# shahruk10/kaldi-tflite

Hardware: AMD Instinct MI355X
Metric: x-vectors/sec (10 s @16 kHz) (higher is better)
Workload: dtype f16mx

## Files before the change

include/ktf_hip.h:

```cpp
#ifndef KTF_HIP_H_
#define KTF_HIP_H_

#include <stddef.h>
#include <stdint.h>

#ifdef __cplusplus
extern "C" {
#endif

#define KTF_OK 0
#define KTF_EINVAL (-1)
#define KTF_ELAUNCH (-2)
#define KTF_EUNSUPPORTED (-3)

#define KTF_F32 0
#define KTF_BF16 1
#define KTF_BF16P 3

#define KTF_GEMM_F32 0
#define KTF_GEMM_BF16 1
#define KTF_GEMM_BF16X3 2
#define KTF_GEMM_F16MX 5
#define KTF_GEMM_BF16X4 6

// ... 104 lines not shown
    int64_t lds_bytes;
    int32_t nsplit;
    int32_t lds_form;
} KtfVcPlan;
int ktf_vad_cmvn_plan(int64_t B, int64_t T, int32_t D, int64_t ldo, KtfVcPlan* plan);
int ktf_cmvn_plan(int64_t T, int32_t D, int64_t ldo, KtfVcPlan* plan);

int ktf_route_short(const int32_t* lens, int64_t B, int32_t min_frames, int32_t* lens_main, int32_t* lens_short, int32_t* host_flag,
                    int32_t seq, void* stream);

typedef struct KtfTdnnDesc {
    int32_t units;
    int32_t din;
    int32_t din_pad;
    int32_t nctx;
    int32_t ctx[16];
    int32_t subsampling;
    int32_t valid;
    int32_t act;
    int32_t gemm;
    int32_t x_dtype, w_dtype, y_dtype;
    int32_t flags;
} KtfTdnnDesc;

#define KTF_TDNN_REF_TILES 1
#define KTF_TDNN_DET_STATS 2
#define KTF_TDNN_K_INTERLEAVED 4
#define KTF_TDNN_W_TILED 8

#define KTF_TDNN_MX_LOADER (1 << 24)

const char* ktf_tdnn_last_kernel(void);


int64_t ktf_tdnn_out_len(int64_t len, const KtfTdnnDesc* d);
int ktf_tdnn_out_lens(const int32_t* lens, int64_t B, const KtfTdnnDesc* d, int32_t* out_lens, void* stream);

int ktf_tdnn(const void* x, int64_t B, int64_t T, int64_t ldx, const int32_t* lens, const KtfTdnnDesc* d,
             const void* w, const void* w_lo, const float* bias, const float* scale, const float* shift,
             void* y, int64_t ldy, int32_t* out_lens, void* stream);

int ktf_tdnn_stats(const void* x, int64_t B, int64_t T, int64_t ldx, const int32_t* lens, const KtfTdnnDesc* d,
                   const void* w, const void* w_lo, const float* bias, const float* scale, const float* shift, double* sums,
                   void* stream);
int ktf_tdnn_split(const void* x_hi, const void* x_lo, int64_t B, int64_t T, int64_t ldx, const int32_t* lens,
                   const KtfTdnnDesc* d, const void* w, const void* w_lo, const float* bias, const float* scale,
                   const float* shift, void* y, void* y_lo, int64_t ldy, int32_t* out_lens, void* stream);
int ktf_tdnn_split_flat(const void* x_hi, const void* x_lo, int64_t B, int64_t T, int64_t ldx, const int32_t* row_starts, const int32_t* row_map,
                        const KtfTdnnDesc* d, const void* w, const void* w_lo, const float* bias, const float* scale,
                        const float* shift, void* y, void* y_lo, int64_t ldy, void* stream);
int64_t ktf_flat_stats_slots(int64_t T);
int64_t ktf_flat_row_map_rows(int64_t B, int64_t T);
int ktf_flat_row_map(const int32_t* row_starts, int64_t B, int64_t T, int32_t* map, void* stream);
int ktf_tdnn_split_flat_stats(const void* x_hi, const void* x_lo, int64_t B, int64_t T, int64_t ldx, const int32_t* row_starts,
                              const int32_t* row_map, const KtfTdnnDesc* d, const void* w, const void* w_lo, const float* bias, const float* scale,
                              const float* shift, double* sums, void* stream);
int ktf_stats_finalize_flat(const double* sums, int64_t slots, const int32_t* row_starts, int64_t T, int64_t B, int32_t D,
                            int32_t include_std, float eps, float* out, int64_t ld_out, void* stream);
int ktf_tdnn_split_stats(const void* x_hi, const void* x_lo, int64_t B, int64_t T, int64_t ldx, const int32_t* lens,
                         const KtfTdnnDesc* d, const void* w, const void* w_lo, const float* bias, const float* scale,
                         const float* shift, double* sums, void* stream);
int ktf_split_bf16(const float* src, int64_t rows, int32_t D, int64_t ld_src, void* hi, void* lo, int64_t ld_dst,
                   void* stream);
int ktf_split_bf16_rows(const float* src, int64_t B, int64_t T, int32_t D, int64_t ld_src, const int32_t* lens, void* hi, void* lo,
                        int64_t ld_dst, void* stream);
int ktf_mx_planes(const float* src, int64_t B, int64_t T, int32_t D, int64_t ld_src, const int32_t* lens, void* xh, void* xl4,
                  void* x4, void* xs, void* stream);
int ktf_tdnn_mx(const void* xh, const void* xl4, const void* x4, const void* xs, int64_t B, int64_t T, const int32_t* lens,
                const KtfTdnnDesc* d, const void* wh, const void* wq, const float* bias, const float* scale, const float* shift,
                void* yh, void* yl4, void* y4, void* ys, float* yf, int64_t ldy, void* stream);
int ktf_tdnn_mx_flat(const void* xh, const void* xl4, const void* x4, const void* xs, int64_t B, int64_t T, const int32_t* row_starts,
                     const int32_t* row_map, const KtfTdnnDesc* d, const void* wh, const void* wq, const float* bias, const float* scale,
                     const float* shift, void* yh, void* yl4, void* y4, void* ys, void* stream);
int ktf_tdnn_mx_flat_stats(const void* xh, const void* xl4, const void* x4, const void* xs, int64_t B, int64_t T, const int32_t* row_starts,
                           const int32_t* row_map, const KtfTdnnDesc* d, const void* wh, const void* wq, const float* bias, const float* scale,
                           const float* shift, double* sums, void* stream);
int ktf_tdnn_mx_stats(const void* xh, const void* xl4, const void* x4, const void* xs, int64_t B, int64_t T, const int32_t* lens,
                      const KtfTdnnDesc* d, const void* wh, const void* wq, const float* bias, const float* scale,
                      const float* shift, double* sums, void* stream);
int ktf_stats_finalize(const double* sums, const int32_t* lens, int64_t T, int64_t B, int32_t D, int32_t include_std,
                       float eps, float* out, int64_t ld_out, void* stream);
int64_t ktf_stats_slots(int64_t T);
int64_t ktf_tdnn_stats_slots(int64_t T, int32_t gemm);
int32_t ktf_tdnn_slot_rows(int32_t gemm);
int64_t ktf_mx_stats_slots(int64_t T, int32_t flags);
int32_t ktf_mx_slot_rows(int32_t flags);
int ktf_stats_finalize_slots(const double* sums, int64_t slots, int32_t slot_rows, const int32_t* lens, int64_t T, int64_t B, int32_t D,
                             int32_t include_std, float eps, float* out, int64_t ld_out, void* stream);

int ktf_activation_f32(float* y, int64_t B, int64_t T, int32_t D, int64_t ld, const int32_t* lens, int32_t act, const float* scale,
                       const float* shift, void* stream);

int ktf_affine_act_f32(const float* x, int64_t rows, int32_t D, int32_t act, const float* scale, const float* shift,
                       float* y, void* stream);
int ktf_convert_pad(const void* src, int32_t src_dtype, int64_t rows, int32_t D, int64_t ld_src, void* dst,
                    int32_t dst_dtype, int64_t ld_dst, void* stream);

int ktf_stats_pool(const void* x, int32_t x_dtype, int64_t B, int64_t T, int32_t D, int64_t ldx,
                   const int32_t* lens, int32_t input_period, int32_t include_std, float eps, float* out,
                   int64_t ld_out, void* stream);
int ktf_stats_pool_windowed_f32(const float* x, int64_t B, int64_t T, int32_t D, int32_t left, int32_t right,
                                int32_t input_period, int32_t output_period, int32_t start, int64_t T_out,
                                int32_t include_std, float eps, float* out, void* stream);

int ktf_xvec_tail_f32(const float* pooled, int64_t ld_pooled, const double* sums, int64_t slots, int32_t slot_rows, const int32_t* lens, int64_t T,
                      int64_t B, int32_t D, int32_t include_std, float eps, const float* W, int64_t ldw, const float* bias,
// ... 187 lines not shown
```

kaldi-tflite_amd/csrc/tdnn_mx.hip:

```cpp
#include "tdnn_mx_common.h"

#define MXP_ROWS 256
__global__ __launch_bounds__(MXP_ROWS) void mx_planes_kernel(const float* __restrict__ src, int64_t T, int64_t ld, int D,
                                                             const int32_t* __restrict__ lens, char* __restrict__ xh,
                                                             char* __restrict__ xl4, char* __restrict__ x4, char* __restrict__ xs) {
    __shared__ float tile[MXP_ROWS * 33];
    const int b = blockIdx.z, c = blockIdx.y, nch = gridDim.y;
    const int64_t t0 = (int64_t)blockIdx.x * MXP_ROWS;
    const int64_t len = lens ? (int64_t)lens[b] : T;
    if (t0 >= len) return;
    const int rows = (int)(len - t0 < MXP_ROWS ? len - t0 : MXP_ROWS);
    const int tid = threadIdx.x;
    const float* base = src + ((int64_t)b * T + t0) * ld + c * 32;
    const bool vec = (ld & 3) == 0 && ((uintptr_t)src & 15) == 0 && c * 32 + 32 <= ld;
#pragma unroll
    for (int k = 0; k < 8; ++k) {
        const int q = k * MXP_ROWS + tid, r = q >> 3, e4 = (q & 7) * 4;
        if (r < rows) {
            float v[4];
            if (vec) {
                const f32x4 t = *reinterpret_cast<const f32x4*>(base + (int64_t)r * ld + e4);
                const int nd = D - (c * 32 + e4);
                v[0] = nd > 0 ? t.x : 0.0f; v[1] = nd > 1 ? t.y : 0.0f; v[2] = nd > 2 ? t.z : 0.0f; v[3] = nd > 3 ? t.w : 0.0f;
            } else {
#pragma unroll
                for (int e = 0; e < 4; ++e) v[e] = (c * 32 + e4 + e < D) ? base[(int64_t)r * ld + e4 + e] : 0.0f;
            }
#pragma unroll
            for (int e = 0; e < 4; ++e) tile[r * 33 + e4 + e] = __builtin_amdgcn_fmed3f(v[e], -65504.0f, 65504.0f);
        }
    }
    __syncthreads();
    const int64_t rec0 = ((int64_t)b * nch + c) * T + t0;
    u32x4 hp[4];
    if (tid < rows) {
        float v[32];
#pragma unroll
        for (int e = 0; e < 32; ++e) v[e] = tile[tid * 33 + e];
        u32x4 l4, h4;
        unsigned sw;
        mx_encode32(v, hp, l4, h4, sw);
        *reinterpret_cast<u32x4*>(xl4 + (rec0 + tid) * 16) = l4;
        *reinterpret_cast<u32x4*>(x4 + (rec0 + tid) * 16) = h4;
        *reinterpret_cast<unsigned*>(xs + (rec0 + tid) * 4) = sw;
    }
    __syncthreads();
    unsigned* himg = reinterpret_cast<unsigned*>(tile);
    if (tid < rows) {
#pragma unroll
        for (int k = 0; k < 4; ++k) *reinterpret_cast<u32x4*>(himg + tid * 20 + k * 4) = hp[k];
    }
    __syncthreads();
#pragma unroll
    for (int k = 0; k < 4; ++k) {
        const int q = k * MXP_ROWS + tid, r = q >> 2;
        if (r < rows)
            *reinterpret_cast<u32x4*>(xh + rec0 * 64 + (int64_t)q * 16) = *reinterpret_cast<const u32x4*>(himg + r * 20 + (q & 3) * 4);
    }
}

extern "C" int ktf_mx_planes(const float* src, int64_t B, int64_t T, int32_t D, int64_t ld_src, const int32_t* lens, void* xh,
                             void* xl4, void* x4, void* xs, void* stream) {
    KTF_REQUIRE(B >= 0 && T >= 0 && D > 0 && ld_src >= D, "ktf_mx_planes: bad size");
    if (B == 0 || T == 0) return KTF_OK;
    KTF_REQUIRE(src && xh && xl4 && x4 && xs, "ktf_mx_planes: null argument");
    const int nch = (D + 31) / 32;
    KTF_REQUIRE(B < 65536 && nch < 65536, "ktf_mx_planes: B and D / 32 must be below 65536");
    hipLaunchKernelGGL(mx_planes_kernel, dim3((unsigned)((T + MXP_ROWS - 1) / MXP_ROWS), (unsigned)nch, (unsigned)B), dim3(MXP_ROWS), 0,
                       (hipStream_t)stream, src, T, ld_src, (int)D, lens, (char*)xh, (char*)xl4, (char*)x4, (char*)xs);
    KTF_CHECK_LAUNCH("ktf_mx_planes");
    return KTF_OK;
}

template <int ACT, int OUT, bool PADK, bool FLAT = false>
__device__ __forceinline__ void mx_tile(const MxParams& p, const int id, int mtiles, int ntiles, int gtiles, double* __restrict__ stats,
                                        unsigned char* rsm) {
    static_assert(!FLAT || OUT != MX_OUT_F32, "flat row tiles: plane output or fused pooling");
#define MX_ARG_BATCH()                                                                                                                     \
    asm volatile("" ::"s"(p.xh), "s"(p.wh), "s"(p.T), "s"(p.nss), "s"(p.nk), "s"(p.nctx), "s"(p.nch_in), "s"(p.ctx_pk[0]), "s"(p.ctx_pk[1]), \
                 "s"(p.t_div_m), "s"(p.t_div_s), "s"(p.start), "s"(p.sub), "s"(p.cut))
    const int xcd = id & 7, slot = id >> 3;
    const int g = (slot / ntiles) * 8 + xcd;
    const int nt = slot - (slot / ntiles) * ntiles;
    if (g >= gtiles) return;
    const int b = FLAT ? 0 : g / mtiles, mt = FLAT ? g : g - b * mtiles;
    const int n0 = nt * 256, t0 = FLAT ? 0 : mt * 256;
    const int tid = threadIdx.x, lane = tid & 63;
    const int wave = __builtin_amdgcn_readfirstlane(tid >> 6);
    const int wm = wave >> 2, wn = wave & 3;
    const int R0 = mt * 256;
    int len, out_len;
    [[maybe_unused]] bool dense = false;
    if constexpr (FLAT) {
        const int total = p.row_starts[mtiles];
        MX_ARG_BATCH();
        if (R0 >= total) return;
        len = (int)p.T;
        out_len = total - R0 < 256 ? total - R0 : 256;
        dense = total == mtiles * len;
    } else {
        len = p.lens ? p.lens[b] : (int)p.T;
        MX_ARG_BATCH();
        out_len = len - p.cut - p.start <= 0 ? 0 : (len - p.cut - p.start + p.sub - 1) / p.sub;
        if (t0 >= out_len) return;
    }
    const int lenm1 = len - 1;
    const int64_t ub = FLAT ? 0 : (int64_t)b * p.nch_in * p.T;
    const int nkp = p.nss * 4;
    const __amdgpu_buffer_rsrc_t r_xh = mx_rsrc_pinned(p.xh + (ub - MX_KQ_BIAS) * 64);
    const __amdgpu_buffer_rsrc_t r_wh = mx_rsrc_pinned(p.wh + (int64_t)nt * nkp * MX_TILE);
    const __amdgpu_buffer_rsrc_t r_wq = mx_rsrc_pinned(p.wq + (int64_t)nt * p.nss * MX_WQ_BLOCK);

    unsigned a_cb[2];
    int a_row[2];
#pragma unroll
    for (int i = 0; i < 2; ++i) {
        const int q = i * 512 + tid;
        const int row = q >> 2;
        a_cb[i] = (unsigned)(((q & 3) ^ ((4 - ((row >> 2) & 3)) & 3)) * 16);
        a_row[i] = p.start + (t0 + row) * p.sub;
    }
    [[maybe_unused]] int a_lm1[2] = {lenm1, lenm1}, s_lm1 = lenm1;
    int s_row = p.start + (t0 + lane + 64 * (wave & 3)) * p.sub;
// ... 428 lines not shown
```

kaldi-tflite_amd/kaldi_tflite_amd/_lib.py:

```python

import ctypes as C
import threading
import os

_HERE = os.path.dirname(os.path.abspath(__file__))
_OVERRIDE = os.environ.get("KTF_LIBRARY") if os.environ.get("KTF_ALLOW_LIBRARY_OVERRIDE") == "1" else None
LIB_PATH = _OVERRIDE or os.path.join(_HERE, "libktf_hip.so")

KTF_F32, KTF_BF16, KTF_BF16P = 0, 1, 3
PAIR = "bf16p"
GEMM_F32, GEMM_BF16, GEMM_BF16X3, GEMM_F16MX, GEMM_BF16X4 = 0, 1, 2, 5, 6
ACT_NONE, ACT_RELU, ACT_SIGMOID, ACT_TANH = 0, 1, 2, 3
(ACT_ELU, ACT_SELU, ACT_SOFTPLUS, ACT_SOFTSIGN, ACT_SWISH, ACT_GELU, ACT_EXPONENTIAL, ACT_HARD_SIGMOID,
 ACT_SOFTMAX) = range(4, 13)
TDNN_REF_TILES, TDNN_DET_STATS, TDNN_K_INTERLEAVED, TDNN_W_TILED = 1, 2, 4, 8
TAIL_SKIP_EMPTY = 1
TDNN_MX_LOADER = 1 << 24

IN_WAV, IN_FRAMES, IN_WINDOWED, IN_WAV_I16 = 0, 1, 2, 3
OUT_FRAMES, OUT_WINDOWED, OUT_FBANK, OUT_MFCC = 0, 1, 2, 3


class KtfBackendError(RuntimeError):
    pass
# ... 28 lines not shown


class VadCfg(C.Structure):
    _fields_ = [("energy_threshold", C.c_float), ("energy_mean_scale", C.c_float), ("proportion_threshold", C.c_float),
                ("frames_context", C.c_int32), ("energy_coeff", C.c_int32)]


class CmvnCfg(C.Structure):
    _fields_ = [("window", C.c_int32), ("norm_vars", C.c_int32), ("valid", C.c_int32), ("reserved", C.c_int32)]


class VcPlan(C.Structure):
    _fields_ = [("pos_ints", C.c_int64), ("stage_floats", C.c_int64), ("bs_floats", C.c_int64), ("col_floats", C.c_int64),
                ("lds_bytes", C.c_int64), ("nsplit", C.c_int32), ("lds_form", C.c_int32)]


class TdnnDesc(C.Structure):
    _fields_ = [("units", C.c_int32), ("din", C.c_int32), ("din_pad", C.c_int32), ("nctx", C.c_int32),
                ("ctx", C.c_int32 * 16), ("subsampling", C.c_int32), ("valid", C.c_int32), ("act", C.c_int32),
                ("gemm", C.c_int32), ("x_dtype", C.c_int32), ("w_dtype", C.c_int32), ("y_dtype", C.c_int32),
                ("flags", C.c_int32)]


_P = C.c_void_p
_i64, _i32, _f32, _u64 = C.c_int64, C.c_int32, C.c_float, C.c_uint64

PROTOTYPES = {
    "ktf_version": (_i32, []),
    "ktf_last_error": (C.c_size_t, [C.c_char_p, C.c_size_t]),
    "ktf_build_id": (C.c_char_p, []),
    "ktf_clock_probe": (C.c_int, [_P, _i64, _P]),
    "ktf_num_frames": (_i64, [_i64, _i32, _i32]),
    "ktf_num_frames_padded": (_i64, [_i64, _i32, _i32, _i32]),
    "ktf_frontend_f32": (C.c_int, [_P, _i64, _i64, _i32, C.POINTER(FrontendCfg), C.POINTER(FrontendTables), _i32, _P, _P, _u64, _P]),
    "ktf_dct_f32": (C.c_int, [_P, _i64, _i32, _i32, _P, _P, _P, _P]),
    "ktf_vad_mask_f32": (C.c_int, [_P, _i64, _i64, _i32, C.POINTER(VadCfg), _P, _P]),
    "ktf_vad_index": (C.c_int, [_P, _i64, _i64, _i32, C.POINTER(VadCfg), _P, _P, _P]),
    "ktf_cmvn_f32": (C.c_int, [_P, _i64, _i64, _i32, _i64, _P, C.POINTER(CmvnCfg), _P, _i64, _P, _P, _P]),
    "ktf_vad_cmvn": (C.c_int, [_P, _i64, _i64, _i32, C.POINTER(VadCfg), C.POINTER(CmvnCfg), _P, _i32, _i64, _P, _P, _P, _P]),
    "ktf_vad_cmvn_plan": (C.c_int, [_i64, _i64, _i32, _i64, C.POINTER(VcPlan)]),
    "ktf_cmvn_plan": (C.c_int, [_i64, _i32, _i64, C.POINTER(VcPlan)]),
    "ktf_route_short": (C.c_int, [_P, _i64, _i32, _P, _P, _P, _i32, _P]),
    "ktf_tdnn_out_len": (_i64, [_i64, C.POINTER(TdnnDesc)]),
    "ktf_tdnn_out_lens": (C.c_int, [_P, _i64, C.POINTER(TdnnDesc), _P, _P]),
    "ktf_tdnn_last_kernel": (C.c_char_p, []),
    "ktf_tdnn": (C.c_int, [_P, _i64, _i64, _i64, _P, C.POINTER(TdnnDesc), _P, _P, _P, _P, _P, _P, _i64, _P, _P]),
    "ktf_tdnn_stats": (C.c_int, [_P, _i64, _i64, _i64, _P, C.POINTER(TdnnDesc), _P, _P, _P, _P, _P, _P, _P]),
    "ktf_tdnn_split": (C.c_int, [_P, _P, _i64, _i64, _i64, _P, C.POINTER(TdnnDesc), _P, _P, _P, _P, _P, _P, _P, _i64, _P, _P]),
    "ktf_tdnn_split_flat": (C.c_int, [_P, _P, _i64, _i64, _i64, _P, _P, C.POINTER(TdnnDesc), _P, _P, _P, _P, _P, _P, _P, _i64, _P]),
    "ktf_tdnn_split_stats": (C.c_int, [_P, _P, _i64, _i64, _i64, _P, C.POINTER(TdnnDesc), _P, _P, _P, _P, _P, _P, _P]),
    "ktf_tdnn_split_flat_stats": (C.c_int, [_P, _P, _i64, _i64, _i64, _P, _P, C.POINTER(TdnnDesc), _P, _P, _P, _P, _P, _P, _P]),
    "ktf_flat_row_map_rows": (_i64, [_i64, _i64]),
    "ktf_flat_row_map": (C.c_int, [_P, _i64, _i64, _P, _P]),
    "ktf_flat_stats_slots": (_i64, [_i64]),
    "ktf_stats_finalize_flat": (C.c_int, [_P, _i64, _P, _i64, _i64, _i32, _i32, _f32, _P, _i64, _P]),
    "ktf_split_bf16": (C.c_int, [_P, _i64, _i32, _i64, _P, _P, _i64, _P]),
    "ktf_split_bf16_rows": (C.c_int, [_P, _i64, _i64, _i32, _i64, _P, _P, _P, _i64, _P]),
    "ktf_mx_planes": (C.c_int, [_P, _i64, _i64, _i32, _i64, _P, _P, _P, _P, _P, _P]),
    "ktf_tdnn_mx": (C.c_int, [_P, _P, _P, _P, _i64, _i64, _P, C.POINTER(TdnnDesc), _P, _P, _P, _P, _P, _P, _P, _P, _P, _P, _i64, _P]),
    "ktf_tdnn_mx_flat": (C.c_int, [_P, _P, _P, _P, _i64, _i64, _P, _P, C.POINTER(TdnnDesc), _P, _P, _P, _P, _P, _P, _P, _P, _P, _P]),
    "ktf_tdnn_mx_flat_stats": (C.c_int, [_P, _P, _P, _P, _i64, _i64, _P, _P, C.POINTER(TdnnDesc), _P, _P, _P, _P, _P, _P, _P]),
    "ktf_tdnn_mx_stats": (C.c_int, [_P, _P, _P, _P, _i64, _i64, _P, C.POINTER(TdnnDesc), _P, _P, _P, _P, _P, _P, _P]),
    "ktf_stats_finalize": (C.c_int, [_P, _P, _i64, _i64, _i32, _i32, _f32, _P, _i64, _P]),
    "ktf_stats_slots": (_i64, [_i64]),
    "ktf_tdnn_stats_slots": (_i64, [_i64, _i32]),
    "ktf_tdnn_slot_rows": (_i32, [_i32]),
    "ktf_mx_stats_slots": (_i64, [_i64, _i32]),
    "ktf_mx_slot_rows": (_i32, [_i32]),
    "ktf_stats_finalize_slots": (C.c_int, [_P, _i64, _i32, _P, _i64, _i64, _i32, _i32, _f32, _P, _i64, _P]),
    "ktf_affine_act_f32": (C.c_int, [_P, _i64, _i32, _i32, _P, _P, _P, _P]),
    "ktf_activation_f32": (C.c_int, [_P, _i64, _i64, _i32, _i64, _P, _i32, _P, _P, _P]),
    "ktf_convert_pad": (C.c_int, [_P, _i32, _i64, _i32, _i64, _P, _i32, _i64, _P]),
    "ktf_stats_pool": (C.c_int, [_P, _i32, _i64, _i64, _i32, _i64, _P, _i32, _i32, _f32, _P, _i64, _P]),
    "ktf_stats_pool_windowed_f32": (C.c_int, [_P, _i64, _i64, _i32, _i32, _i32, _i32, _i32, _i32, _i64, _i32, _f32, _P, _P]),
    "ktf_xvec_post_f32": (C.c_int, [_P, _i64, _i32, _i32, _P, _P, _P, _P, _P]),
    "ktf_xvec_tail_f32": (C.c_int, [_P, _i64, _P, _i64, _i32, _P, _i64, _i64, _i32, _i32, _f32, _P, _i64, _P, _i32, _P, _P, _P, _i32, _P, _P, _P, _P, _i32, _i32, _P]),
    "ktf_plda_f64": (C.c_int, [_P, _i64, _i32, _P, _P, _P, _i32, _i32, _P, _P, _P]),
    "ktf_plda_f32": (C.c_int, [_P, _i64, _i32, _P, _P, _P, _i32, _i32, _P, _P, _P]),
    "ktf_plda_score_f64": (C.c_int, [_P, _i64, _P, _i64, _i32, _P, _P, _P]),
    "ktf_plda_score_f32": (C.c_int, [_P, _i64, _P, _i64, _i32, _P, _P, _P]),
    "ktf_spk_mean_f32": (C.c_int, [_P, _i64, _i32, _P, _i64, _P, _i64, _P, _P, _P]),
    "ktf_plda_transform_n_f64": (C.c_int, [_P, _i64, _i32, _P, _P, _P, _P, _i32, _i32, _P, _P]),
    "ktf_plda_transform_n_f32": (C.c_int, [_P, _i64, _i32, _P, _P, _P, _P, _i32, _i32, _P, _P]),
    "ktf_plda_score_n_f64": (C.c_int, [_P, _i64, _P, _i64, _i32, _P, _P, _P, _P]),
    "ktf_plda_score_n_f32": (C.c_int, [_P, _i64, _P, _i64, _i32, _P, _P, _P, _P]),
    "ktf_plda_trials_workspace_bytes": (_i64, [_i64, _i64, _i32, _i32]),
    "ktf_plda_trials_f64": (C.c_int, [_P, _i64, _P, _i64, _i32, _P, _P, _P, _i64, _P, _P, C.c_size_t, _P]),
    "ktf_plda_trials_f32": (C.c_int, [_P, _i64, _P, _i64, _i32, _P, _P, _P, _i64, _P, _P, C.c_size_t, _P]),
    "ktf_topn_stats_f64": (C.c_int, [_P, _i64, _i64, _i64, _i32, _P, _P, _P]),
    "ktf_topn_stats_f32": (C.c_int, [_P, _i64, _i64, _i64, _i32, _P, _P, _P]),
    "ktf_plda_cohort_workspace_bytes": (_i64, [_i64, _i64, _i32, _i32]),
    "ktf_plda_cohort_stats_f64": (C.c_int, [_P, _i64, _P, _i64, _i32, _P, _P, _i32, _i32, _P, _P, _P, C.c_size_t, _P]),
    "ktf_plda_cohort_stats_f32": (C.c_int, [_P, _i64, _P, _i64, _i32, _P, _P, _i32, _i32, _P, _P, _P, C.c_size_t, _P]),
    "ktf_plda_dense_workspace_bytes": (_i64, [_P, _i32, _i32, C.c_double]),
    "ktf_plda_dense_f64": (C.c_int, [_P, _i64, _i32, _P, _P, _i32, C.c_double, _P, _P, _P, _P, _P, _P, _i32, _i32, _P, _P, _P,
                                     C.c_size_t, _P, _P]),
    "ktf_plda_dense_f32": (C.c_int, [_P, _i64, _i32, _P, _P, _i32, C.c_double, _P, _P, _P, _P, _P, _P, _i32, _i32, _P, _P, _P,
                                     C.c_size_t, _P, _P]),
    "ktf_ahc_workspace_bytes": (_i64, [_P, _i32, _i32]),
    "ktf_ahc_f64": (C.c_int, [_P, _P, _P, _i32, _i32, C.c_double, _P, C.c_double, _P, _P, _P, C.c_size_t, _P]),
    "ktf_ahc_f32": (C.c_int, [_P, _P, _P, _i32, _i32, C.c_double, _P, C.c_double, _P, _P, _P, C.c_size_t, _P]),
    "ktf_diar_segments": (C.c_int, [_P, _i32, _P, _P, _i32, C.POINTER(VadCfg), _P, _P, _P]),
    "ktf_diar_windows": (C.c_int, [_P, _P, _P, _i32, _i32, _i32, _i32, _P, _P, _P]),
    "ktf_diar_compact": (C.c_int, [_P, _P, _P, _P, _P, _i32, _i64, _i64, _P, _P, _P]),
    "ktf_diar_segment_cmn": (C.c_int, [_P, _i32, _P, _P, _i32, _P, _i64, C.POINTER(CmvnCfg), _P, _P, _P]),
    "ktf_diar_gather": (C.c_int, [_P, _i32, _P, _P, _i32, _P, _i64, _i64, _i64, _i32, _P, _i32, _i32, _P, _P]),
# ... 188 lines not shown
```

kaldi-tflite_amd/kaldi_tflite_amd/models.py:

```python

import math
import os
import threading

import numpy as np
import torch

from . import _lib as L
from . import ops
from .io import KaldiNnet3Reader, ReadKaldiArray
from .layers import TDNN, BatchNorm, CMVN, Framing, MFCC, ReLU, StatsPooling, VAD, _GEMM, WEIGHTS_EPOCH, _f32_rows
from .mx import Planes


class Input:

    def __init__(self, shape=None, batch_size=None, name="input"):
        self.shape = (batch_size,) + tuple(shape)
        self.name = name


_LAYER_KINDS = (
    (("affine", "tdnn"), TDNN, "{}.affine", True),
    (("relu",), ReLU, "{}.relu", False),
# ... 191 lines not shown
                steps.append(("stats", l))
                pooled = True
                i += 1
            elif isinstance(l, (ReLU, BatchNorm)):
                steps.append(("eltwise", l))
                i += 1
            else:
                return None
        return steps

    def batch_gemm(self, B, T, mode=None):
        return self._batch_route(B, T, mode)[0]

    def _batch_route(self, B, T, mode=None):
        if mode is None:
            mode = self.gemm
            if T < self.frames_floor(mode):
                mode = self.SHORT_MODE.get(mode, "f32")
        gemm = _GEMM[mode]
        if gemm != L.GEMM_F32 and -(-(B * T) // 256) < self.min_tiles.get(mode, 0):
            return L.GEMM_F32, bool(self.small_tile_pairs)
        return gemm, False

    @property
    def _ws(self):
        return getattr(self._tl, "ws", None) or self._ws_own

    @_ws.setter
    def _ws(self, ws):
        self._tl.ws = None if ws is self._ws_own else ws

    def _mx_use_loader(self, B, T):
        if self.mx_loader is not None:
            return bool(self.mx_loader)
        rounds = lambda wgs: -(-wgs // 256)
        cost_256 = rounds(2 * B * ((T + 255) // 256)) * 256
        cost_loader = rounds(2 * ((B * T + 191) // 192)) * 192 * 1.05
        return cost_loader < cost_256

    def _flat_tiles(self, l, B, T, ldx):
        if not (self.flat_rows and B * T > 0 and l.padding == "SAME" and l.subsamplingFactor == 1 and l.activation in (None, "linear", "relu")
                and B <= 4095 and B * T * ldx * 2 < 2 ** 32):
            return False
        return bool(5 * (-(-T // 16)) < 4 * (-(-T // 256)) * 16 or (self.flat_rows_long and _fewer_flat_tiles(B, T)))

    def _tail_step(self, steps):
        if len(steps) >= 2 and steps[-1][0] == "tdnn" and steps[-2][0] == "stats":
            _, l, relu, bn = steps[-1]
            if (not relu and bn is None and l.activation in (None, "linear") and l.kernelWidth == 1 and l.padding == "SAME"
                    and l.subsamplingFactor == 1 and l.units <= 512 and l.inputDim <= 3072):
                return len(steps) - 1
        return -1

    def run_ragged(self, x, lens=None, defer_tail=False, mode=None):
        steps = self._plan()
        if steps is None:
            raise NotImplementedError("this layer stack is not supported by the fused ragged runner")
        self._ws.enter(x.device)
        gemm, pairs = self._batch_route(x.shape[0], x.shape[1], mode=mode)
        tail_at = self._tail_step(steps) if defer_tail else -1
        c = _RunState(self._ws, x, lens, gemm, pairs, tail_at, steps[tail_at][1] if tail_at >= 0 else None)
        for si, st in enumerate(steps):
            if c.skip:
                c.skip = False
                continue
            if si == tail_at and c.deferred is not None:
                return c.deferred
            nxt = steps[si + 1] if si + 1 < len(steps) else None
            out_role = f"act{si & 1}" + ("s" if c.pooled else "") + ("p" if st[0] == "tdnn" and st[1].units % 32 else "")
            own = can_pool = False
            if st[0] == "tdnn":
                _, l, relu, _ = st
                if relu and l.activation not in (None, "linear"):
                    raise ValueError("cannot fuse a ReLU after a TDNN that already has an activation")
                can_pool = (self.fuse_stats and not c.pooled and nxt is not None and nxt[0] == "stats" and
                            nxt[1].inputPeriod == 1 and l.units > 128 and l.padding == "SAME" and l.subsamplingFactor == 1)
                if not c.pooled:
                    l.warn_fallback(gemm, relu)
                    own = l.effective_gemm(gemm, relu) == gemm
            if own and gemm == L.GEMM_F16MX:
                self._step_mx(c, si, st, nxt, can_pool, out_role)
                continue
            if c.mxp is not None:
                raise RuntimeError("internal: MX planes reached a layer that cannot read them")
            if c.pending_bn is not None:
                raise RuntimeError("internal: a deferred BatchNorm reached a layer that cannot fold it")
            if own and gemm == L.GEMM_BF16X3 and self.split_planes and l.units > 128:
                self._step_planes(c, si, st, nxt, can_pool, out_role)
                continue
            if c.planes is not None:
                raise RuntimeError("internal: split planes reached a layer that cannot read them")
            if st[0] == "tdnn":
                self._step_generic(c, si, st, nxt, can_pool, out_role)
            elif st[0] == "stats":
                self._step_stats(c, si, st[1])
            else:
                c.x = st[1](c.x.to(torch.float32).contiguous())
        if c.pooled:
            return c.x.reshape(c.x.shape[1], 1, c.x.shape[2])
        return c.x

    def _step_mx(self, c, si, st, nxt, can_pool, out_role):
        _, l, relu, bn = st
        if c.mxp is None:
            B, T, D = c.x.shape
            src = _f32_rows(c.x)
            c.mxp = Planes.buffers(c.ws.get, "mx_in", B, T, D, c.dev)
            ops.mx_planes(src, D, c.lens, c.mxp)
        B, T, _ = c.mxp.shape
        fold, c.pending_bn = c.pending_bn, None
        plain = l.padding == "SAME" and l.subsamplingFactor == 1
        use_loader = plain and self._mx_use_loader(B, T)
        wh, wq, bias = l.device_weights_mx(c.dev, fold=fold, kernel="loader" if use_loader else "tile")
        mxf = L.TDNN_MX_LOADER if use_loader else 0
# ... 405 lines not shown
        ops.vad_cmvn(mfcc, self.vad.cfg(), self.cmvn.cfg(), feats, lens, idx, work)
        return mfcc, feats[:, :, :D], lens

    def features(self, inputs):
        mfcc, feats, lens = self._features(inputs)
        return mfcc.clone(), feats.clone(), lens.clone()

    def extract_stream(self, host_batches, depth=3):
        L.require_gpu()
        dev = ops.default_device()
        compute = torch.cuda.current_stream(dev)
        copy = torch.cuda.Stream(device=dev)
        bufs, free = [None] * depth, [None] * depth
        for i, hb in enumerate(host_batches):
            hb = hb if isinstance(hb, torch.Tensor) else torch.as_tensor(hb)
            k = i % depth
            with torch.cuda.stream(copy):
                if free[k] is not None:
                    copy.wait_event(free[k])
                if bufs[k] is None or bufs[k].shape != hb.shape or bufs[k].dtype != hb.dtype:
                    bufs[k] = torch.empty(hb.shape, dtype=hb.dtype, device=dev)
                bufs[k].copy_(hb, non_blocking=True)
                ready = torch.cuda.Event()
                ready.record(copy)
            compute.wait_event(ready)
            y = self(bufs[k])
            free[k] = torch.cuda.Event()
            free[k].record(compute)
            yield y

    def _extract(self, inputs, out=None):
        y, feats, lens = self._extract_routed(inputs, out)
        if (self.verify_fraction > 0 and self.gemm in self.xvec.SHORT_MODE and not torch.cuda.is_current_stream_capturing()
                and not self._warming_for_capture):
            self._verify(feats, lens, y)
        return y

    def _extract_routed(self, inputs, out=None):
        _, feats, lens = self._features(inputs)
        self.last_lens = lens
        return self._route_xvectors(feats, lens, out), feats, lens

    def _route_xvectors(self, feats, lens, out=None, raw=None):
        B, T = feats.shape[0], feats.shape[1]
        seq = self.xvec
        nshort = seq.frames_floor(seq.gemm)
        if not (self.route_short_utterances and nshort > 0 and T >= nshort and seq.gemm in seq.SHORT_MODE
                and seq.batch_gemm(B, T) == _GEMM[seq.gemm]):
            return self._xvectors(feats, lens, out, raw=raw)
        ws = self._ws
        lens_main = ws.get("lens_main", (B,), torch.int32, feats.device, padded=False)
        lens_short = ws.get("lens_short", (B,), torch.int32, feats.device, padded=False)
        capturing = torch.cuda.is_current_stream_capturing()
        if capturing:
            ops.route_short(lens, nshort, lens_main, lens_short)
        else:
            tl = self._tl
            if getattr(tl, "short_flag", None) is None:
                tl.short_flag = torch.zeros(2, dtype=torch.int32).pin_memory()
                tl.short_seq = 0
            tl.short_seq = (tl.short_seq % 0x3FFFFFFF) + 1
            ops.route_short(lens, nshort, lens_main, lens_short, tl.short_flag, tl.short_seq)
        y = self._xvectors(feats, lens_main, out, raw=raw)
        if not capturing:
            self.last_short_count = self._await_short_count(feats.device)
            if self.last_short_count == 0 and not self._warming_for_capture:
                return y
        short_mode = seq.SHORT_MODE[seq.gemm]
        if self._tail_fusable() and self.fuse_tail:
            self._xvectors(feats, lens_short, y, mode=short_mode, skip_empty=True, raw=raw)
        else:
            raw2 = None if raw is None else torch.empty_like(raw)
            y2 = self._xvectors(feats, lens_short, None, mode=short_mode, raw=raw2)
            y.copy_(torch.where((lens_short > 0)[:, None], y2, y))
            if raw is not None:
                raw.copy_(torch.where((lens_short > 0)[:, None], raw2, raw))
        return y

    def _await_short_count(self, dev):
        import time
        flag, want = self._tl.short_flag, self._tl.short_seq
        t0 = time.perf_counter()
        spins = 0
        while int(flag[1]) != want:
            spins += 1
            if spins > 200:
                time.sleep(0 if spins < 2000 else 50e-6)
            if time.perf_counter() - t0 > 2.0:
                torch.cuda.current_stream(dev).synchronize()
                if int(flag[1]) != want:
                    raise RuntimeError("ktf_route_short: the short-utterance count did not reach the host")
                break
        return int(flag[0])

    def _xvectors(self, feats, lens, out=None, mode=None, skip_empty=False, raw=None):
        one_launch = self.fuse_tail and self._tail_fusable() and (skip_empty or feats.shape[0] < self.fuse_tail_below or
                                                                  self.xvec.batch_gemm(feats.shape[0], feats.shape[1], mode=mode) == L.GEMM_F32)
        if skip_empty and not one_launch:
            raise RuntimeError("internal: skip_empty needs the fused tail")
        h = self.xvec.run_ragged(feats, lens, defer_tail=one_launch, mode=mode)
        dev = feats.device
        mean, A, off = self._post_params(dev)
        if isinstance(h, DeferredTail):
            t = h
            if t.layer.units == A.shape[0]:
                w6, _, b6 = t.layer.device_weights(dev, L.GEMM_F32)
                B = t.B
                group = max(1, min(32, (B * 64) // 2048))
                if t.sums is not None and (B > 8 or t.slots > 4):
                    sbuf = self.xvec._ws.get("pooled", (B, ops.round_up((2 if t.include_std else 1) * t.D, 32)), torch.float32, dev)
                    ops.stats_finalize(t.sums, t.lens, t.T, t.D, t.include_std, t.eps, sbuf, slots=t.slots, slot_rows=t.slot_rows)
                    t.pooled, t.sums = sbuf, None
                odim = A.shape[1]
                ws = self._ws
                partial = ws.get("tail_partial", (B, 64, odim), torch.float32, dev, padded=False)
                counters = ws.get("tail_cnt", (B,), torch.int32, dev, padded=True)
                if out is None:
                    out = torch.empty((B, odim), dtype=torch.float32, device=dev)
                return ops.xvec_tail(t.pooled, t.sums, t.slots, t.lens, t.T, t.D, t.include_std, t.eps, w6, b6, t.layer.units, mean, A, off,
                                     partial, counters, out, h_out=raw, group=group, slot_rows=t.slot_rows, skip_empty=skip_empty)
            raise ValueError(f"LDA input dim {A.shape[0]} != embedding dim {t.layer.units}")
        B = h.shape[0]
        h2 = h.reshape(B, h.shape[-1])
        if not h2.is_contiguous():
            h2 = h2.contiguous()
        if raw is not None:
            raw.copy_(h2)
        return ops.xvec_post(h2, mean, A, off, out=out)

    def _post_params(self, dev):
        key = str(dev)
        if key not in self._post_dev:
            self._post_dev[key] = (ops.to_device_f32(self.xvecGlobalMean, dev), ops.to_device_f32(self.ldaMat, dev),
                                   ops.to_device_f32(self.ldaOffset.reshape(-1), dev))
        return self._post_dev[key]

    def embeddings(self, wavs):
        L.require_gpu()
        units = self.ldaMat.shape[0]
        if hasattr(wavs, "shape") and len(wavs.shape) == 2 and wavs.shape[0] == 0:
            return torch.empty((0, units), dtype=torch.float32, device=ops.default_device())
        dev = wavs.device if (isinstance(wavs, torch.Tensor) and wavs.is_cuda) else ops.default_device()
        with L.launch_scope(dev):
            _, feats, lens = self._features(wavs)
            self.last_lens = lens
            raw = torch.empty((feats.shape[0], units), dtype=torch.float32, device=feats.device)
            self._route_xvectors(feats, lens, raw=raw)
        return raw

    def postprocess(self, raw):
        L.require_gpu()
        x = raw if isinstance(raw, torch.Tensor) else torch.as_tensor(np.asarray(raw, np.float32))
        if not x.is_cuda:
# ... 202 lines not shown
```

kaldi-tflite_amd/kaldi_tflite_amd/ops.py:

```python

import ctypes as C

import numpy as np
import torch

from . import _lib as L


def _dev(device=None):
    L.require_gpu()
    return torch.device(device) if device is not None else torch.device("cuda", torch.cuda.current_device())


def default_device():
    return _dev(None)


def to_device_f32(x, device=None):
    dev = _dev(device)
    if isinstance(x, torch.Tensor):
        return x.to(device=dev, dtype=torch.float32).contiguous()
    return torch.as_tensor(np.ascontiguousarray(np.asarray(x, dtype=np.float32)), device=dev)


# ... 509 lines not shown
    lib = L.load()
    with L.on_device(src.device):
        if lens is None:
            rc = lib.ktf_split_bf16(L.ptr(src), src.shape[0] * src.shape[1], D, src.stride(1), L.ptr(planes[0]), L.ptr(planes[1]), planes.shape[-1],
                                    L.stream_ptr())
        else:
            rc = lib.ktf_split_bf16_rows(L.ptr(src), src.shape[0], src.shape[1], D, src.stride(1), L.ptr(lens), L.ptr(planes[0]), L.ptr(planes[1]),
                                         planes.shape[-1], L.stream_ptr())
    L.check(rc, "ktf_split_bf16")
    return planes


def _planes(xp):
    if xp.dim() != 4 or xp.shape[0] != 2:
        raise ValueError(f"expected a (2, B, T, ldx) pair of bf16 planes, got shape {tuple(xp.shape)}")
    return xp[0], xp[1], xp.shape[1], xp.shape[2], xp.stride(2)


def tdnn_split(xp, lens, desc, w, w_lo, bias, scale, shift, y, y_lo=None, out_lens=None):
    lib = L.load()
    hi, lo, B, T, ldx = _planes(xp)
    with L.on_device(xp.device):
        rc = lib.ktf_tdnn_split(L.ptr(hi), L.ptr(lo), B, T, ldx, L.ptr(lens), C.byref(desc), L.ptr(w), L.ptr(w_lo),
                                L.ptr(bias), L.ptr(scale), L.ptr(shift), L.ptr(y), L.ptr(y_lo), y.stride(1), L.ptr(out_lens),
                                L.stream_ptr())
    L.check(rc, "ktf_tdnn_split")
    return y


def row_starts(lens, B, T, out):
    if lens is None:
        out[1:] = torch.arange(1, B + 1, dtype=torch.int32, device=out.device) * int(T)
    else:
        torch.cumsum(lens, 0, dtype=torch.int32, out=out[1:])
    return out


class FlatRows:

    def __init__(self, starts, map=None):
        self.starts, self.map = starts, map


def flat_rows(lens, B, T, get):
    lib = L.load()
    starts = row_starts(lens, B, T, get("row_starts", (B + 1,), torch.int32))
    table = get("row_map", (int(lib.ktf_flat_row_map_rows(B, T)), 4), torch.int32)
    with L.on_device(starts.device):
        rc = lib.ktf_flat_row_map(L.ptr(starts), B, T, L.ptr(table), L.stream_ptr())
    L.check(rc, "ktf_flat_row_map")
    return FlatRows(starts, table)


def _flat(starts):
    return (starts.starts, starts.map) if isinstance(starts, FlatRows) else (starts, None)


def tdnn_split_flat(xp, starts, desc, w, w_lo, bias, scale, shift, y, y_lo=None):
    lib = L.load()
    hi, lo, B, T, ldx = _planes(xp)
    starts, rmap = _flat(starts)
    with L.on_device(xp.device):
        rc = lib.ktf_tdnn_split_flat(L.ptr(hi), L.ptr(lo), B, T, ldx, L.ptr(starts), L.ptr(rmap), C.byref(desc), L.ptr(w), L.ptr(w_lo),
                                     L.ptr(bias), L.ptr(scale), L.ptr(shift), L.ptr(y), L.ptr(y_lo), y.stride(1), L.stream_ptr())
    L.check(rc, "ktf_tdnn_split_flat")
    return y


def tdnn_split_stats(xp, lens, desc, w, w_lo, bias, scale, shift, sums, zero=True):
    lib = L.load()
    hi, lo, B, T, ldx = _planes(xp)
    with L.on_device(xp.device):
        if zero:
            sums.zero_()
        rc = lib.ktf_tdnn_split_stats(L.ptr(hi), L.ptr(lo), B, T, ldx, L.ptr(lens), C.byref(desc), L.ptr(w),
                                      L.ptr(w_lo), L.ptr(bias), L.ptr(scale), L.ptr(shift), L.ptr(sums), L.stream_ptr())
    L.check(rc, "ktf_tdnn_split_stats")
    return sums


def flat_stats_slots(T):
    return int(L.load().ktf_flat_stats_slots(int(T)))


def tdnn_split_flat_stats(xp, starts, desc, w, w_lo, bias, scale, shift, sums, zero=False):
    lib = L.load()
    hi, lo, B, T, ldx = _planes(xp)
    starts, rmap = _flat(starts)
    with L.on_device(xp.device):
        if zero:
            sums.zero_()
        rc = lib.ktf_tdnn_split_flat_stats(L.ptr(hi), L.ptr(lo), B, T, ldx, L.ptr(starts), L.ptr(rmap), C.byref(desc), L.ptr(w), L.ptr(w_lo),
                                           L.ptr(bias), L.ptr(scale), L.ptr(shift), L.ptr(sums), L.stream_ptr())
    L.check(rc, "ktf_tdnn_split_flat_stats")
    return sums


def stats_finalize_flat(sums, starts, T, D, include_std, eps, out, slots):
    lib = L.load()
    B = sums.shape[0]
    starts, _ = _flat(starts)
    with L.on_device(sums.device):
        rc = lib.ktf_stats_finalize_flat(L.ptr(sums), slots, L.ptr(starts), T, B, D, int(include_std), eps, L.ptr(out), out.stride(0),
                                         L.stream_ptr())
    L.check(rc, "ktf_stats_finalize_flat")
    return out
# ... 648 lines not shown
```

Before: 111,800.

## Fuse short-utterance routing, flat row map and input MX planes into one launch

Adds a kernel that routes short utterances, builds the flat row starts and row map, and encodes the first layer's MX input planes in a single launch. Previously these were separate kernels, route_short, flat_rows and mx_planes. The Python path hands the precomputed rows and planes into run_ragged when the f16mx flat-row route applies. This cuts launch count and serialized small kernels, but each row-map workgroup redundantly recomputes the prefix sum over all lengths, and B is limited to 4095.

```diff
diff --git a/include/ktf_hip.h b/include/ktf_hip.h
--- a/include/ktf_hip.h
+++ b/include/ktf_hip.h
@@ -180,6 +180,9 @@
 int64_t ktf_flat_stats_slots(int64_t T);
 int64_t ktf_flat_row_map_rows(int64_t B, int64_t T);
 int ktf_flat_row_map(const int32_t* row_starts, int64_t B, int64_t T, int32_t* map, void* stream);
+int ktf_route_short_rows(const int32_t* lens, int64_t B, int64_t T, int32_t min_frames, int32_t* lens_main, int32_t* lens_short,
+                         int32_t* host_flag, int32_t seq, int32_t* row_starts, int32_t* map, const float* src, int32_t D, int64_t ld_src,
+                         void* xh, void* xl4, void* x4, void* xs, void* stream);
 int ktf_tdnn_split_flat_stats(const void* x_hi, const void* x_lo, int64_t B, int64_t T, int64_t ldx, const int32_t* row_starts,
                               const int32_t* row_map, const KtfTdnnDesc* d, const void* w, const void* w_lo, const float* bias, const float* scale,
                               const float* shift, double* sums, void* stream);
diff --git a/kaldi-tflite_amd/csrc/tdnn_mx.hip b/kaldi-tflite_amd/csrc/tdnn_mx.hip
--- a/kaldi-tflite_amd/csrc/tdnn_mx.hip
+++ b/kaldi-tflite_amd/csrc/tdnn_mx.hip
@@ -1,13 +1,9 @@
 #include "tdnn_mx_common.h"
 
 #define MXP_ROWS 256
-__global__ __launch_bounds__(MXP_ROWS) void mx_planes_kernel(const float* __restrict__ src, int64_t T, int64_t ld, int D,
-                                                             const int32_t* __restrict__ lens, char* __restrict__ xh,
-                                                             char* __restrict__ xl4, char* __restrict__ x4, char* __restrict__ xs) {
-    __shared__ float tile[MXP_ROWS * 33];
-    const int b = blockIdx.z, c = blockIdx.y, nch = gridDim.y;
-    const int64_t t0 = (int64_t)blockIdx.x * MXP_ROWS;
-    const int64_t len = lens ? (int64_t)lens[b] : T;
+__device__ __forceinline__ void mx_planes_block(float* tile, int b, int c, int nch, int64_t t0, int64_t len, const float* __restrict__ src,
+                                                int64_t T, int64_t ld, int D, char* __restrict__ xh, char* __restrict__ xl4,
+                                                char* __restrict__ x4, char* __restrict__ xs) {
     if (t0 >= len) return;
     const int rows = (int)(len - t0 < MXP_ROWS ? len - t0 : MXP_ROWS);
     const int tid = threadIdx.x;
@@ -57,6 +53,14 @@
         if (r < rows)
             *reinterpret_cast<u32x4*>(xh + rec0 * 64 + (int64_t)q * 16) = *reinterpret_cast<const u32x4*>(himg + r * 20 + (q & 3) * 4);
     }
+}
+
+__global__ __launch_bounds__(MXP_ROWS) void mx_planes_kernel(const float* __restrict__ src, int64_t T, int64_t ld, int D,
+                                                             const int32_t* __restrict__ lens, char* __restrict__ xh,
+                                                             char* __restrict__ xl4, char* __restrict__ x4, char* __restrict__ xs) {
+    __shared__ float tile[MXP_ROWS * 33];
+    const int b = blockIdx.z;
+    mx_planes_block(tile, b, blockIdx.y, gridDim.y, (int64_t)blockIdx.x * MXP_ROWS, lens ? (int64_t)lens[b] : T, src, T, ld, D, xh, xl4, x4, xs);
 }
 
 extern "C" int ktf_mx_planes(const float* src, int64_t B, int64_t T, int32_t D, int64_t ld_src, const int32_t* lens, void* xh,
@@ -69,6 +73,113 @@
     hipLaunchKernelGGL(mx_planes_kernel, dim3((unsigned)((T + MXP_ROWS - 1) / MXP_ROWS), (unsigned)nch, (unsigned)B), dim3(MXP_ROWS), 0,
                        (hipStream_t)stream, src, T, ld_src, (int)D, lens, (char*)xh, (char*)xl4, (char*)x4, (char*)xs);
     KTF_CHECK_LAUNCH("ktf_mx_planes");
+    return KTF_OK;
+}
+
+#define RR_PER 16
+#define RR_TILES 4
+static_assert(MXP_ROWS * 33 >= MXP_ROWS * RR_PER + 16, "the plane tile also holds the prefix sums");
+__global__ __launch_bounds__(MXP_ROWS) void route_rows_kernel(const int32_t* __restrict__ lens, int B, int T, int32_t min_frames,
+                                                              int32_t* __restrict__ lens_main, int32_t* __restrict__ lens_short,
+                                                              int32_t* host_flag, int32_t seq, int32_t* __restrict__ row_starts,
+                                                              i32x4* __restrict__ map, int64_t rows, int row_wgs, const float* __restrict__ src,
+                                                              int64_t ld, int D, char* __restrict__ xh, char* __restrict__ xl4,
+                                                              char* __restrict__ x4, char* __restrict__ xs) {
+    __shared__ float tile[MXP_ROWS * 33];
+    if ((int)blockIdx.x >= row_wgs) {
+        const int nt = (T + MXP_ROWS - 1) / MXP_ROWS, nch = (D + 31) / 32;
+        const int j = (int)blockIdx.x - row_wgs;
+        const int b = j / (nt * nch), c = (j / nt) % nch;
+        const int len = lens[b];
+        mx_planes_block(tile, b, c, nch, (int64_t)(j % nt) * MXP_ROWS, len >= min_frames ? len : 0, src, T, ld, D, xh, xl4, x4, xs);
+        return;
+    }
+    int* rs = reinterpret_cast<int*>(tile);
+    int* wtot = rs + MXP_ROWS * RR_PER;
+    int* wshort = wtot + MXP_ROWS / 64;
+    const int tid = threadIdx.x, lane = tid & 63, wave = tid >> 6;
+    const bool first = blockIdx.x == 0;
+    int lm[RR_PER];
+    int s = 0, ns = 0;
+#pragma unroll
+    for (int k = 0; k < RR_PER; ++k) {
+        const int b = tid * RR_PER + k;
+        const int len = b < B ? lens[b] : 0;
+        const bool is_short = len > 0 && len < min_frames;
+        lm[k] = len >= min_frames ? len : 0;
+        if (first && b < B) {
+            lens_main[b] = lm[k];
+            lens_short[b] = is_short ? len : 0;
+        }
+        s += lm[k];
+        ns += is_short ? 1 : 0;
+    }
+    int incl = s;
+#pragma unroll
+    for (int o = 1; o < 64; o <<= 1) {
+        const int up = __shfl_up(incl, o, 64);
+        if (lane >= o) incl += up;
+    }
+#pragma unroll
+    for (int o = 32; o > 0; o >>= 1) ns += __shfl_xor(ns, o, 64);
+    if (lane == 63) wtot[wave] = incl;
+    if (lane == 0) wshort[wave] = ns;
+    __syncthreads();
+    int run = incl - s;
+    for (int w = 0; w < wave; ++w) run += wtot[w];
+#pragma unroll
+    for (int k = 0; k < RR_PER; ++k) {
+        const int b = tid * RR_PER + k;
+        if (b <= B) {
+            rs[b] = run;
+            if (first) row_starts[b] = run;
+        }
+        run += lm[k];
+    }
+    if (first && tid == 0 && host_flag) {
+        int tot = 0;
+        for (int w = 0; w < MXP_ROWS / 64; ++w) tot += wshort[w];
+        __hip_atomic_store(host_flag, tot, __ATOMIC_RELAXED, __HIP_MEMORY_SCOPE_SYSTEM);
+        __hip_atomic_store(host_flag + 1, seq, __ATOMIC_RELEASE, __HIP_MEMORY_SCOPE_SYSTEM);
+    }
+    __syncthreads();
+    const int total = rs[B];
+#pragma unroll
+    for (int i = 0; i < RR_TILES; ++i) {
+        const int64_t R = ((int64_t)blockIdx.x * RR_TILES + i) * 256 + tid;
+        if (R >= rows) break;
+        i32x4 e = {-1, 0, 1, 0};
+        if (R < total) {
+            int lo = 0, hi = B - 1;
+            while (lo < hi) {
+                const int mid = (lo + hi + 1) >> 1;
+                if (rs[mid] <= R) lo = mid; else hi = mid - 1;
+            }
+            const int s0 = rs[lo], t = (int)R - s0;
+            e = i32x4{lo * T + t, t, rs[lo + 1] - s0, lo};
+        }
+        map[R] = e;
+    }
+}
+
+extern "C" int ktf_route_short_rows(const int32_t* lens, int64_t B, int64_t T, int32_t min_frames, int32_t* lens_main, int32_t* lens_short,
+                                    int32_t* host_flag, int32_t seq, int32_t* row_starts, int32_t* map, const float* src, int32_t D,
+                                    int64_t ld_src, void* xh, void* xl4, void* x4, void* xs, void* stream) {
+    KTF_REQUIRE(B > 0 && T > 0 && B <= 4095 && B * T < (1ll << 31) && min_frames >= 0, "ktf_route_short_rows: bad sizes");
+    KTF_REQUIRE(lens && lens_main && lens_short && row_starts && map, "ktf_route_short_rows: null argument");
+    const int64_t rows = ktf_flat_row_map_rows(B, T);
+    const int row_wgs = ktf_cdiv(rows, 256 * RR_TILES);
+    int64_t plane_wgs = 0;
+    if (src) {
+        KTF_REQUIRE(D > 0 && ld_src >= D, "ktf_route_short_rows: bad size");
+        KTF_REQUIRE(xh && xl4 && x4 && xs, "ktf_route_short_rows: null plane");
+        plane_wgs = B * ((D + 31) / 32) * ((T + MXP_ROWS - 1) / MXP_ROWS);
+        KTF_REQUIRE(row_wgs + plane_wgs < (1ll << 31), "ktf_route_short_rows: too many workgroups");
+    }
+    hipLaunchKernelGGL(route_rows_kernel, dim3((unsigned)(row_wgs + plane_wgs)), dim3(MXP_ROWS), 0, (hipStream_t)stream, lens, (int)B, (int)T,
+                       min_frames, lens_main, lens_short, host_flag, seq, row_starts, reinterpret_cast<i32x4*>(map), rows, row_wgs, src, ld_src,
+                       (int)D, (char*)xh, (char*)xl4, (char*)x4, (char*)xs);
+    KTF_CHECK_LAUNCH("ktf_route_short_rows");
     return KTF_OK;
 }
 
diff --git a/kaldi-tflite_amd/kaldi_tflite_amd/_lib.py b/kaldi-tflite_amd/kaldi_tflite_amd/_lib.py
--- a/kaldi-tflite_amd/kaldi_tflite_amd/_lib.py
+++ b/kaldi-tflite_amd/kaldi_tflite_amd/_lib.py
@@ -104,6 +104,7 @@
     "ktf_tdnn_split_flat_stats": (C.c_int, [_P, _P, _i64, _i64, _i64, _P, _P, C.POINTER(TdnnDesc), _P, _P, _P, _P, _P, _P, _P]),
     "ktf_flat_row_map_rows": (_i64, [_i64, _i64]),
     "ktf_flat_row_map": (C.c_int, [_P, _i64, _i64, _P, _P]),
+    "ktf_route_short_rows": (C.c_int, [_P, _i64, _i64, _i32, _P, _P, _P, _i32, _P, _P, _P, _i32, _i64, _P, _P, _P, _P, _P]),
     "ktf_flat_stats_slots": (_i64, [_i64]),
     "ktf_stats_finalize_flat": (C.c_int, [_P, _i64, _P, _i64, _i64, _i32, _i32, _f32, _P, _i64, _P]),
     "ktf_split_bf16": (C.c_int, [_P, _i64, _i32, _i64, _P, _P, _i64, _P]),
diff --git a/kaldi-tflite_amd/kaldi_tflite_amd/models.py b/kaldi-tflite_amd/kaldi_tflite_amd/models.py
--- a/kaldi-tflite_amd/kaldi_tflite_amd/models.py
+++ b/kaldi-tflite_amd/kaldi_tflite_amd/models.py
@@ -267,7 +267,18 @@
                 return len(steps) - 1
         return -1
 
-    def run_ragged(self, x, lens=None, defer_tail=False, mode=None):
+    def premade_rows_pay(self, B, T):
+        return bool(self.gemm == "f16mx" and self._batch_route(B, T)[0] == L.GEMM_F16MX and self.mx_flat_rows and B * T > 0 and B <= 4095
+                    and B * T < 2 ** 31 and not self._mx_use_loader(B, T) and _fewer_flat_tiles(B, T))
+
+    def first_layer_reads_planes(self):
+        steps = self._plan()
+        if not steps or steps[0][0] != "tdnn":
+            return False
+        _, l, relu, _ = steps[0]
+        return not (relu and l.activation not in (None, "linear")) and l.effective_gemm(L.GEMM_F16MX, relu) == L.GEMM_F16MX
+
+    def run_ragged(self, x, lens=None, defer_tail=False, mode=None, rows=None, planes=None):
         steps = self._plan()
         if steps is None:
             raise NotImplementedError("this layer stack is not supported by the fused ragged runner")
@@ -275,6 +286,12 @@
         gemm, pairs = self._batch_route(x.shape[0], x.shape[1], mode=mode)
         tail_at = self._tail_step(steps) if defer_tail else -1
         c = _RunState(self._ws, x, lens, gemm, pairs, tail_at, steps[tail_at][1] if tail_at >= 0 else None)
+        if rows is not None:
+            c._rows, c._rows_for = rows, (x.shape[0], x.shape[1])
+        if planes is not None:
+            if gemm != L.GEMM_F16MX or not self.first_layer_reads_planes():
+                raise RuntimeError("internal: input planes handed to a run whose first layer does not read them")
+            c.mxp = planes
         for si, st in enumerate(steps):
             if c.skip:
                 c.skip = False
@@ -786,16 +803,25 @@
         lens_main = ws.get("lens_main", (B,), torch.int32, feats.device, padded=False)
         lens_short = ws.get("lens_short", (B,), torch.int32, feats.device, padded=False)
         capturing = torch.cuda.is_current_stream_capturing()
-        if capturing:
-            ops.route_short(lens, nshort, lens_main, lens_short)
-        else:
+        flag = ()
+        if not capturing:
             tl = self._tl
             if getattr(tl, "short_flag", None) is None:
                 tl.short_flag = torch.zeros(2, dtype=torch.int32).pin_memory()
                 tl.short_seq = 0
             tl.short_seq = (tl.short_seq % 0x3FFFFFFF) + 1
-            ops.route_short(lens, nshort, lens_main, lens_short, tl.short_flag, tl.short_seq)
-        y = self._xvectors(feats, lens_main, out, raw=raw)
+            flag = (tl.short_flag, tl.short_seq)
+        rows = planes = None
+        if seq.premade_rows_pay(B, T):
+            get = lambda role, shape, dt, device=feats.device, padded=False: ws.get("route_" + role, shape, dt, device, padded=False)
+            src = D = None
+            if seq.first_layer_reads_planes():
+                src, D = _f32_rows(feats), feats.shape[2]
+                planes = Planes.buffers(get, "mx_in", B, T, D, feats.device)
+            rows = ops.route_short_rows(lens, T, nshort, lens_main, lens_short, get, *(flag or (None, 0)), src=src, D=D or 0, planes=planes)
+        else:
+            ops.route_short(lens, nshort, lens_main, lens_short, *flag)
+        y = self._xvectors(feats, lens_main, out, raw=raw, rows=rows, planes=planes)
         if not capturing:
             self.last_short_count = self._await_short_count(feats.device)
             if self.last_short_count == 0 and not self._warming_for_capture:
@@ -827,12 +853,12 @@
                 break
         return int(flag[0])
 
-    def _xvectors(self, feats, lens, out=None, mode=None, skip_empty=False, raw=None):
+    def _xvectors(self, feats, lens, out=None, mode=None, skip_empty=False, raw=None, rows=None, planes=None):
         one_launch = self.fuse_tail and self._tail_fusable() and (skip_empty or feats.shape[0] < self.fuse_tail_below or
                                                                   self.xvec.batch_gemm(feats.shape[0], feats.shape[1], mode=mode) == L.GEMM_F32)
         if skip_empty and not one_launch:
             raise RuntimeError("internal: skip_empty needs the fused tail")
-        h = self.xvec.run_ragged(feats, lens, defer_tail=one_launch, mode=mode)
+        h = self.xvec.run_ragged(feats, lens, defer_tail=one_launch, mode=mode, rows=rows, planes=planes)
         dev = feats.device
         mean, A, off = self._post_params(dev)
         if isinstance(h, DeferredTail):
diff --git a/kaldi-tflite_amd/kaldi_tflite_amd/ops.py b/kaldi-tflite_amd/kaldi_tflite_amd/ops.py
--- a/kaldi-tflite_amd/kaldi_tflite_amd/ops.py
+++ b/kaldi-tflite_amd/kaldi_tflite_amd/ops.py
@@ -585,6 +585,24 @@
     return FlatRows(starts, table)
 
 
+def route_short_rows(lens, T, min_frames, lens_main, lens_short, get, host_flag=None, seq=0, src=None, D=0, planes=None):
+    lib = L.load()
+    B = lens.shape[0]
+    starts = get("row_starts", (B + 1,), torch.int32)
+    table = get("row_map", (int(lib.ktf_flat_row_map_rows(B, T)), 4), torch.int32)
+    if src is not None and (src.shape[0] != B or src.shape[1] != T):
+        raise ValueError(f"src {tuple(src.shape)} is not a (B = {B}, T = {T}, ld) batch")
+    with L.on_device(lens.device):
+        rc = lib.ktf_route_short_rows(L.ptr(lens), B, int(T), int(min_frames), L.ptr(lens_main), L.ptr(lens_short),
+                                      host_flag.data_ptr() if host_flag is not None else None, int(seq), L.ptr(starts), L.ptr(table),
+                                      L.ptr(src), int(D), src.stride(1) if src is not None else 0,
+                                      L.ptr(planes.xh) if src is not None else None, L.ptr(planes.xl4) if src is not None else None,
+                                      L.ptr(planes.x4) if src is not None else None, L.ptr(planes.xs) if src is not None else None,
+                                      L.stream_ptr())
+    L.check(rc, "ktf_route_short_rows")
+    return FlatRows(starts, table)
+
+
 def _flat(starts):
     return (starts.starts, starts.map) if isinstance(starts, FlatRows) else (starts, None)
 
```

Result: no change. 111,900, median of 2 (+0.1%).
